# megvii-research/basedet

Measured on AMD Instinct MI355X. Metric: images/sec training RetinaNet-R50-FPN 1333x800, higher is better.
Workload: dtype bf16; 1 GPU; retinanet_r50_800x1344 train step (fwd+bwd+allreduce+SGD), DummyLoader boxes, random-init weights, inputs resident in HBM; per_gpu_batch=16, global_batch=16, parallelism=dp1

## Files before the change

basedet_amd/csrc/conv_wgrad.hip:

```cpp
#include <vector>
#include "common.h"

namespace {

constexpr int TILE = 128;
constexpr int ROW_PITCH = 288;
constexpr int MAX_SEG = BD_MAX_SEGS;

struct WSeg {
    int m_start;
    int Ho, Wo, per_img;
    float inv_per_img, inv_wo;
    int Hi, Wi, in_off, out_off;
};

struct WgradParams {
    const bf16_raw* x;
    const bf16_raw* g;
    float* slab;
    int Cin, Cout, R, S, stride, pad;
    int M, nseg;
    int in_pix_per_img, out_pix_per_img;
    int ci_tiles, co_tiles, splits, steps_per_split, total_steps;
    WSeg seg[MAX_SEG];
};

__device__ __forceinline__ void fast_divmod(int n, int d, float inv, int& q, int& r) {
    q = (int)((float)n * inv);
    r = n - q * d;
    if (r < 0) { --q; r += d; }
    else if (r >= d) { ++q; r -= d; }
}

template <int BKP, bool USE_TR>
__global__ __launch_bounds__(256) void conv_wgrad_kernel(const WgradParams p) {
    constexpr int PASSES = BKP / 16;
    constexpr int TILE_BYTES = BKP * ROW_PITCH;
    extern __shared__ __attribute__((aligned(16))) unsigned char smem[];

    const int tid = threadIdx.x;
    const int lane = tid & 63;
    const int wave = tid >> 6;
    const int wci = wave >> 1;
    const int wco = wave & 1;

    const int nwg = gridDim.x;
    int bid = blockIdx.x;
    {
        const int q = nwg >> 3, r = nwg & 7, xcd = bid & 7;
        bid = (xcd < r ? xcd * (q + 1) : r * (q + 1) + (xcd - r) * q) + (bid >> 3);
    }
    const int RS = p.R * p.S;
    const int tiles_per_split = RS * p.ci_tiles * p.co_tiles;
    const int split = bid / tiles_per_split;
    int t = bid - split * tiles_per_split;
    const int tap = t / (p.ci_tiles * p.co_tiles);
    t -= tap * (p.ci_tiles * p.co_tiles);
    const int ci_tile = t / p.co_tiles;
    const int co_tile = t - ci_tile * p.co_tiles;
    const int ci0 = ci_tile * TILE, co0 = co_tile * TILE;
    const int tap_r = tap / p.S, tap_s = tap - tap_r * p.S;

    const int step_begin = split * p.steps_per_split;
    int step_end = step_begin + p.steps_per_split;
    if (step_end > p.total_steps) step_end = p.total_steps;

    const int chunk = tid & 15;
    const int row0 = tid >> 4;
    const bool ci_ok = ci0 + chunk * 8 < p.Cin;
    const bool co_ok = co0 + chunk * 8 < p.Cout;

    u32x4_t rx[PASSES], rg[PASSES];

    auto stage_load = [&](int step) {
#pragma unroll
        for (int i = 0; i < PASSES; ++i) {
            const int m = step * BKP + row0 + i * 16;
            u32x4_t vx = {0u, 0u, 0u, 0u}, vg = {0u, 0u, 0u, 0u};
            if (m < p.M) {
                int s = 0;
#pragma unroll
                for (int k = 1; k < MAX_SEG; ++k)
                    if (k < p.nseg && m >= p.seg[k].m_start) s = k;
                const WSeg sg = p.seg[s];
                int n, rem, oy, ox;
                fast_divmod(m - sg.m_start, sg.per_img, sg.inv_per_img, n, rem);
                fast_divmod(rem, sg.Wo, sg.inv_wo, oy, ox);
                if (co_ok) {
                    const long long gp = (long long)n * p.out_pix_per_img + sg.out_off + oy * sg.Wo + ox;
                    vg = *reinterpret_cast<const u32x4_t*>(p.g + gp * p.Cout + co0 + chunk * 8);
                }
                const int sy = oy * p.stride - p.pad + tap_r, sx = ox * p.stride - p.pad + tap_s;
                if (ci_ok && sy >= 0 && sx >= 0 && sy < sg.Hi && sx < sg.Wi) {
                    const long long xp = (long long)n * p.in_pix_per_img + sg.in_off + sy * sg.Wi + sx;
                    vx = *reinterpret_cast<const u32x4_t*>(p.x + xp * p.Cin + ci0 + chunk * 8);
                }
            }
            rx[i] = vx; rg[i] = vg;
        }
    };
    auto stage_write = [&](int buf) {
        unsigned char* Xt = smem + buf * 2 * TILE_BYTES;
        unsigned char* Gt = Xt + TILE_BYTES;
#pragma unroll
        for (int i = 0; i < PASSES; ++i) {
            const int row = row0 + i * 16;
            *reinterpret_cast<u32x4_t*>(Xt + row * ROW_PITCH + chunk * 16) = rx[i];
            *reinterpret_cast<u32x4_t*>(Gt + row * ROW_PITCH + chunk * 16) = rg[i];
        }
    };

    f32x4_t acc[4][4];
#pragma unroll
    for (int i = 0; i < 4; ++i)
#pragma unroll
        for (int j = 0; j < 4; ++j) acc[i][j] = (f32x4_t){0.f, 0.f, 0.f, 0.f};

    const int g4 = lane >> 4, idx = lane & 15;
    const int prow_base = 16 * (g4 >> 1) + 4 * (g4 & 1);
    const int tr_q = idx >> 2, tr_p = idx & 3;

    auto load_frag = [&](const unsigned char* tile, int kk, int cbase) -> bf16x8_t {
        bf16x8_t f;
        if constexpr (USE_TR) {
            const unsigned char* a0 = tile + (kk * 32 + prow_base + tr_q) * ROW_PITCH + (cbase + 4 * tr_p) * 2;
            s16x4_t lo = __builtin_amdgcn_ds_read_tr16_b64_v4i16((__attribute__((address_space(3))) s16x4_t*)(a0));
            s16x4_t hi = __builtin_amdgcn_ds_read_tr16_b64_v4i16((__attribute__((address_space(3))) s16x4_t*)(a0 + 8 * ROW_PITCH));
            typedef __attribute__((ext_vector_type(8))) short s16x8_t;
            s16x8_t v = {lo[0], lo[1], lo[2], lo[3], hi[0], hi[1], hi[2], hi[3]};
            f = __builtin_bit_cast(bf16x8_t, v);
        } else {
            typedef __attribute__((ext_vector_type(8))) short s16x8_t;
            s16x8_t v;
#pragma unroll
            for (int j = 0; j < 8; ++j) {
                const int prow = kk * 32 + prow_base + (j & 3) + 8 * (j >> 2);
                v[j] = *reinterpret_cast<const short*>(tile + prow * ROW_PITCH + (cbase + idx) * 2);
            }
            f = __builtin_bit_cast(bf16x8_t, v);
        }
        return f;
    };

    auto compute = [&](int buf) {
        const unsigned char* Xt = smem + buf * 2 * TILE_BYTES;
        const unsigned char* Gt = Xt + TILE_BYTES;
#pragma unroll
        for (int kk = 0; kk < BKP / 32; ++kk) {
            bf16x8_t a[4], b[4];
#pragma unroll
            for (int i = 0; i < 4; ++i) a[i] = load_frag(Xt, kk, wci * 64 + i * 16);
#pragma unroll
            for (int j = 0; j < 4; ++j) b[j] = load_frag(Gt, kk, wco * 64 + j * 16);
#pragma unroll
            for (int i = 0; i < 4; ++i)
#pragma unroll
                for (int j = 0; j < 4; ++j)
                    acc[i][j] = __builtin_amdgcn_mfma_f32_16x16x32_bf16(a[i], b[j], acc[i][j], 0, 0, 0);
        }
    };

    if (step_begin < step_end) {
        stage_load(step_begin);
        stage_write(0);
    }
    __syncthreads();
    int cur = 0;
    for (int st = step_begin; st < step_end; ++st) {
        const bool more = st + 1 < step_end;
        if (more) stage_load(st + 1);
        compute(cur);
        if (more) stage_write(cur ^ 1);
        __syncthreads();
        cur ^= 1;
    }

    float* slab = p.slab + (long long)split * p.Cout * RS * p.Cin;
#pragma unroll
    for (int j = 0; j < 4; ++j) {
        const int co = co0 + wco * 64 + j * 16 + idx;
        if (co >= p.Cout) continue;
#pragma unroll
        for (int i = 0; i < 4; ++i) {
            const int ci = ci0 + wci * 64 + i * 16 + g4 * 4;
            if (ci >= p.Cin) continue;
            *reinterpret_cast<f32x4_t*>(slab + ((long long)co * RS + tap) * p.Cin + ci) = acc[i][j];
        }
    }
}

}
#include "wgrad_reduce.h"
namespace {

__global__ __launch_bounds__(256) void wgrad_batch_reduce_kernel(const BdRedBatch b) {
    __shared__ f32x4_t red[4][64];
    int ei = 0;
#pragma unroll 1
    for (int k = 1; k < b.count; ++k)
        if ((int)blockIdx.x >= b.e[k].block_begin) ei = k;
    const BdRedEntry& en = b.e[ei];
    const int tx = threadIdx.x & 63, ty = threadIdx.x >> 6;
    const long long e = (long long)((int)blockIdx.x - en.block_begin) * 64 + tx;
    const long long n4 = en.n4;
    f32x4_t s = {0.f, 0.f, 0.f, 0.f};
    if (e < n4) {
        const long long stride = n4 * 4;
        const float* src = en.slab + e * 4;
        const int splits = en.splits;
        int k = ty;
        for (; k + 12 < splits; k += 16) {
            const f32x4_t v0 = *reinterpret_cast<const f32x4_t*>(src + (long long)k * stride);
            const f32x4_t v1 = *reinterpret_cast<const f32x4_t*>(src + (long long)(k + 4) * stride);
            const f32x4_t v2 = *reinterpret_cast<const f32x4_t*>(src + (long long)(k + 8) * stride);
            const f32x4_t v3 = *reinterpret_cast<const f32x4_t*>(src + (long long)(k + 12) * stride);
            s += v0; s += v1; s += v2; s += v3;
        }
        for (; k < splits; k += 4) s += *reinterpret_cast<const f32x4_t*>(src + (long long)k * stride);
    }
    red[ty][tx] = s;
    __syncthreads();
    if (ty != 0 || e >= n4) return;
    f32x4_t t = red[0][tx];
    t += red[1][tx]; t += red[2][tx]; t += red[3][tx];
    long long idx;
    int row;
    if (en.kind == 0) {
        idx = e * 4;
        row = (int)(idx / en.row_len);
    } else {
        const int regs = en.regs;
        const long long per_tile = 8ll * regs * 64;
        const int tile = (int)(e / per_tile);
        int r = (int)(e - tile * per_tile);
        const int wave = r / (regs * 64);
        r -= wave * (regs * 64);
        const int reg = r >> 6, lane = r & 63;
        const int ci_tile = tile / en.co_tiles, co_tile = tile - ci_tile * en.co_tiles;
        int co, ci, tap = 0, taps = 1;
        if (en.kind == 1) {
            tap = reg >> 2; taps = 9;
            co = co_tile * en.tco + (wave >> 2) * 64 + (reg & 3) * 16 + (lane & 15);
            ci = ci_tile * en.tci + (wave & 3) * 16 + (lane >> 4) * 4;
        } else {
            const int i = reg / en.fj, j = reg - i * en.fj;
            const int wco_n = en.tco / (16 * en.fj);
            const int wci = wave / wco_n, wco = wave - wci * wco_n;
            co = co_tile * en.tco + (wco * en.fj + j) * 16 + (lane & 15);
            ci = ci_tile * en.tci + (wci * en.fi + i) * 16 + (lane >> 4) * 4;
        }
        if (co >= en.Cout || ci >= en.Cin) return;
        idx = ((long long)co * taps + tap) * en.Cin + ci;
        row = co;
    }
    float* d = en.dw + idx;
    if (en.row_scale) t *= en.row_scale[row];
    if (en.accumulate) t += *reinterpret_cast<const f32x4_t*>(d);
    *reinterpret_cast<f32x4_t*>(d) = t;
}

int launch_batch(const BdRedEntry* entries, int count, hipStream_t stream) {
    for (int base = 0; base < count; base += BD_RED_MAX) {
        BdRedBatch b{};
        b.count = count - base < BD_RED_MAX ? count - base : BD_RED_MAX;
        int blocks = 0;
        for (int k = 0; k < b.count; ++k) {
            b.e[k] = entries[base + k];
            b.e[k].block_begin = blocks;
            blocks += (int)cdiv64(b.e[k].n4, 64);
        }
        if (blocks > 0) hipLaunchKernelGGL(wgrad_batch_reduce_kernel, dim3(blocks), dim3(256), 0, stream, b);
    }
    return 0;
}

BdRedEntry plain_entry(const float* slab, int splits, long long n, int row_len, const float* row_scale, float* dw, int accumulate) {
    BdRedEntry e{};
    e.slab = slab; e.dw = dw; e.row_scale = row_scale; e.kind = 0; e.splits = splits; e.accumulate = accumulate;
    e.n4 = (int)(n / 4); e.row_len = row_len;
    return e;
}

struct Plan { int ci_tiles, co_tiles, splits, steps_per_split, total_steps; long long M; };

constexpr int BKP_DEFAULT = 64;
BD_KNOB int g_wgrad_use_tr = 1;
BD_KNOB int g_wgrad_use_3x3 = 1;
BD_KNOB int g_wgrad_use_ring = 1;

bool is_3x3s1(const bd_conv_desc* d) {
    if (!(d->R == 3 && d->S == 3 && (d->stride == 1 || d->stride == 2) && d->pad == 1)) return false;
    if ((long long)d->N * d->in_pix_per_img * d->Cin * 2 >= 0x7fffffffll || (long long)d->N * d->out_pix_per_img * d->Cout * 2 >= 0x7fffffffll)
        return false;
    for (int s = 0; s < d->nseg; ++s)
        if ((d->Hi[s] - 1) / d->stride + 1 != d->Ho[s] || (d->Wi[s] - 1) / d->stride + 1 != d->Wo[s]) return false;
    return true;
}

Plan make_plan(const bd_conv_desc* d) {
    Plan pl;
    long long M = 0;
    for (int s = 0; s < d->nseg; ++s) M += (long long)d->N * d->Ho[s] * d->Wo[s];
    pl.M = M;
    pl.ci_tiles = cdiv(d->Cin, TILE);
    pl.co_tiles = cdiv(d->Cout, TILE);
    pl.total_steps = (int)cdiv64(M, BKP_DEFAULT);
    const int tiles = d->R * d->S * pl.ci_tiles * pl.co_tiles;
    int splits = 1024 / tiles;
    if (splits < 1) splits = 1;
    const int max_splits = pl.total_steps / 4 > 0 ? pl.total_steps / 4 : 1;
    if (splits > max_splits) splits = max_splits;
    pl.steps_per_split = cdiv(pl.total_steps, splits);
    pl.splits = cdiv(pl.total_steps, pl.steps_per_split);
    return pl;
}

}

int bd_wgrad1x1_splits(const bd_conv_desc* d);
int bd_wgrad1x1_launch(const bd_conv_desc* d, const void* x, const void* g, float* slab, int* splits_out, hipStream_t stream);
int bd_wgrad3x3_splits(const bd_conv_desc* d, int* total_patches_out, int* patches_per_img_out);
int bd_wgrad3x3_launch(const bd_conv_desc* d, const void* x, const void* g, float* slab, float* csum, int* splits_out, hipStream_t stream);
bool bd_wgrad3x3r_eligible(const bd_conv_desc* d);
size_t bd_wgrad3x3r_slab_bytes(const bd_conv_desc* d, int* splits_out);
int bd_wgrad3x3r_launch(const bd_conv_desc* d, const void* x, const void* g, float* slab, float* csum, const int* gflags, int* splits_out,
                        hipStream_t stream);
int bd_wgrad3x3r_gskip_patches(const bd_conv_desc* d);
void bd_gskip_scan(const bd_conv_desc* d, const void* g, int ph, int pw, int* mask, hipStream_t stream);
void bd_wgrad3x3r_entry(const bd_conv_desc* d, BdRedEntry* e);
bool bd_wgrad1x1r_eligible(const bd_conv_desc* d);
size_t bd_wgrad1x1r_slab_bytes(const bd_conv_desc* d, int* splits_out);
int bd_wgrad1x1r_launch(const bd_conv_desc* d, const void* x, const void* g, float* slab, int* splits_out, hipStream_t stream);
void bd_wgrad1x1r_entry(const bd_conv_desc* d, BdRedEntry* e);

int bd_route_wgrad(int use_tr) {
    g_wgrad_use_tr = use_tr & 1;
    g_wgrad_use_3x3 = (use_tr & 2) ? 0 : 1;
    g_wgrad_use_ring = (use_tr & 4) ? 0 : 1;
    if (!(use_tr & 1)) g_wgrad_use_3x3 = 0;
    return BD_OK;
}

void bd_wgrad_reduce_launch(const float* slab, int splits, long long n, int row_len, const float* row_scale, float* dw, int accumulate,
                            hipStream_t stream) {
    const BdRedEntry e = plain_entry(slab, splits, n, row_len, row_scale, dw, accumulate);
    launch_batch(&e, 1, stream);
}

namespace {
size_t align256(size_t v) { return (v + 255) & ~size_t(255); }
int gskip_patches(const bd_conv_desc* d) {
    return d->gskip && bd_wgrad3x3r_eligible(d) ? bd_wgrad3x3r_gskip_patches(d) : 0;
}
size_t wgrad_ws_base(const bd_conv_desc* d);
}

extern "C" size_t bd_conv2d_wgrad_workspace_bytes(const bd_conv_desc* d) {
    BdRouteScope rs__(d);
    if (rs__.rc != BD_OK) return 0;
    if (!d || d->nseg < 1 || d->nseg > BD_MAX_SEGS) return 0;
    const size_t base = wgrad_ws_base(d);
    const int gp = gskip_patches(d);
    return gp > 0 ? align256(base) + (size_t)gp * sizeof(int) : base;
}

namespace {
size_t wgrad_ws_base(const bd_conv_desc* d) {
    const Plan pl = make_plan(d);
    size_t splits = (size_t)pl.splits;
    if (is_3x3s1(d)) {
        const size_t s3 = (size_t)bd_wgrad3x3_splits(d, nullptr, nullptr);
        if (s3 > splits) splits = s3;
    }
    if (d->R == 1 && d->S == 1 && d->pad == 0) {
        const size_t s1 = (size_t)bd_wgrad1x1_splits(d);
        if (s1 > splits) splits = s1;
    }
    size_t bytes = splits * d->Cout * d->R * d->S * d->Cin * sizeof(float);
    if (bd_wgrad3x3r_eligible(d)) {
        const size_t r = bd_wgrad3x3r_slab_bytes(d, nullptr);
        if (r > bytes) bytes = r;
    }
    if (bd_wgrad1x1r_eligible(d)) {
        const size_t r = bd_wgrad1x1r_slab_bytes(d, nullptr);
        if (r > bytes) bytes = r;
    }
    return bytes;
}
}

extern "C" size_t bd_colsum_workspace_bytes(int C);
extern "C" int bd_colsum_bf16(const void* g, int N, int64_t pix_per_img, int64_t off, int64_t cnt, int C, float* out, int accumulate,
                              void* ws, size_t ws_bytes, bd_stream_t stream);
struct bd_wgrad_queue { std::vector<BdRedEntry> entries; };
static int wgrad_impl(const bd_conv_desc* d, const void* x, const void* g, const float* row_scale, float* dw, float* dbias,
                      int accumulate, void* ws, size_t ws_bytes, bd_stream_t stream, bd_wgrad_queue* q);

extern "C" size_t bd_conv2d_wgrad_bias_workspace_bytes(const bd_conv_desc* d) {
    BdRouteScope rs__(d);
    if (rs__.rc != BD_OK) return 0;
    const size_t w = bd_conv2d_wgrad_workspace_bytes(d);
    if (!w) return 0;
    size_t extra = bd_colsum_workspace_bytes(d->Cout);
    if (is_3x3s1(d)) {
        const size_t s3 = (size_t)bd_wgrad3x3_splits(d, nullptr, nullptr) * d->Cout * sizeof(float);
        if (s3 > extra) extra = s3;
    }
    if (bd_wgrad3x3r_eligible(d)) {
        int sr = 1;
        (void)bd_wgrad3x3r_slab_bytes(d, &sr);
        const size_t s3 = (size_t)sr * d->Cout * sizeof(float);
        if (s3 > extra) extra = s3;
    }
    return align256(w) + extra;
}

extern "C" int bd_conv2d_wgrad_bias(const bd_conv_desc* d, const void* x, const void* g, const float* row_scale, float* dw,
                                    float* dbias, int accumulate, void* ws, size_t ws_bytes, bd_stream_t stream) {
    BD_ROUTE(d);
    BD_REQUIRE(dbias, "conv2d_wgrad_bias: null bias gradient");
    BD_REQUIRE(d != nullptr, "conv2d_wgrad_bias: null descriptor");
    const size_t need = bd_conv2d_wgrad_bias_workspace_bytes(d);
    if (ws_bytes < need) {
        bd_set_error("conv2d_wgrad_bias: workspace %zu < required %zu bytes", ws_bytes, need);
        return BD_EWORKSPACE;
    }
    return wgrad_impl(d, x, g, row_scale, dw, dbias, accumulate, ws, ws_bytes, stream, nullptr);
}

extern "C" int bd_conv2d_wgrad(const bd_conv_desc* d, const void* x, const void* g, const float* row_scale,
                               float* dw, int accumulate, void* ws, size_t ws_bytes, bd_stream_t stream) {
    BD_ROUTE(d);
    return wgrad_impl(d, x, g, row_scale, dw, nullptr, accumulate, ws, ws_bytes, stream, nullptr);
}

extern "C" int bd_wgrad_queue_create(bd_wgrad_queue_t* out) {
    BD_REQUIRE(out != nullptr, "bd_wgrad_queue_create: null argument");
    *out = new bd_wgrad_queue();
    return BD_OK;
}
extern "C" int bd_wgrad_queue_destroy(bd_wgrad_queue_t q) {
    delete q;
    return BD_OK;
}
extern "C" int bd_wgrad_queue_pending(bd_wgrad_queue_t q) { return q ? (int)q->entries.size() : 0; }
extern "C" int bd_conv2d_wgrad_queued(bd_wgrad_queue_t q, const bd_conv_desc* d, const void* x, const void* g, const float* row_scale, float* dw,
                                      float* dbias, int accumulate, void* ws, size_t ws_bytes, bd_stream_t stream) {
    BD_ROUTE(d);
    BD_REQUIRE(q != nullptr, "bd_conv2d_wgrad_queued: null queue");
    if (dbias) {
        BD_REQUIRE(d != nullptr, "conv2d_wgrad_queued: null descriptor");
        const size_t need = bd_conv2d_wgrad_bias_workspace_bytes(d);
        if (ws_bytes < need) {
            bd_set_error("conv2d_wgrad_queued: workspace %zu < required %zu bytes", ws_bytes, need);
            return BD_EWORKSPACE;
        }
    }
    return wgrad_impl(d, x, g, row_scale, dw, dbias, accumulate, ws, ws_bytes, stream, q);
}
extern "C" int bd_wgrad_queue_flush(bd_wgrad_queue_t q, bd_stream_t stream) {
    BD_REQUIRE(q != nullptr, "bd_wgrad_queue_flush: null queue");
    if (q->entries.empty()) return BD_OK;
    launch_batch(q->entries.data(), (int)q->entries.size(), (hipStream_t)stream);
    q->entries.clear();
    BD_CHECK_LAUNCH("bd_wgrad_queue_flush");
    return BD_OK;
}

static int wgrad_impl(const bd_conv_desc* d, const void* x, const void* g, const float* row_scale, float* dw, float* dbias,
                      int accumulate, void* ws, size_t ws_bytes, bd_stream_t stream, bd_wgrad_queue* q) {
    BD_REQUIRE(d && x && g && dw && ws, "conv2d_wgrad: null pointer");
    BD_REQUIRE(d->nseg >= 1 && d->nseg <= BD_MAX_SEGS, "conv2d_wgrad: nseg out of range");
    BD_REQUIRE(d->Cin % 8 == 0 && d->Cout % 8 == 0, "conv2d_wgrad: Cin=%d / Cout=%d must be multiples of 8", d->Cin, d->Cout);
    const Plan pl = make_plan(d);
    BD_REQUIRE(pl.M < (1ll << 24), "conv2d_wgrad: %lld pixels exceed the 2^24 fast-division range", pl.M);
    const size_t need = bd_conv2d_wgrad_workspace_bytes(d);
    if (ws_bytes < need) {
        bd_set_error("conv2d_wgrad: workspace %zu < required %zu bytes", ws_bytes, need);
        return BD_EWORKSPACE;
    }
    unsigned char* extra = (unsigned char*)ws + align256(need);
    auto bias_fallback = [&]() -> int {
        long long dense = 0;
        bool packed = true;
        for (int s = 0; s < d->nseg; ++s) { packed = packed && d->out_off[s] == dense; dense += (long long)d->Ho[s] * d->Wo[s]; }
        if (packed && dense == d->out_pix_per_img)
            return bd_colsum_bf16(g, 1, 0, 0, (int64_t)d->N * dense, d->Cout, dbias, accumulate, extra, bd_colsum_workspace_bytes(d->Cout), stream);
        for (int s = 0; s < d->nseg; ++s) {
            const int e = bd_colsum_bf16(g, d->N, d->out_pix_per_img, d->out_off[s], (int64_t)d->Ho[s] * d->Wo[s], d->Cout, dbias,
                                         (s > 0 || accumulate) ? 1 : 0, extra, bd_colsum_workspace_bytes(d->Cout), stream);
            if (e != BD_OK) return e;
        }
        return BD_OK;
    };
    auto finish = [&](const BdRedEntry& we, int splits, bool fused_csum) -> int {
        BdRedEntry es[2] = {we, {}};
        int n = 1;
        if (dbias && fused_csum) es[n++] = plain_entry((const float*)extra, splits, d->Cout, 1, nullptr, dbias, accumulate);
        if (q) {
            for (int k = 0; k < n; ++k) q->entries.push_back(es[k]);
        } else {
            launch_batch(es, n, (hipStream_t)stream);
            BD_CHECK_LAUNCH("bd_conv2d_wgrad(reduce)");
        }
        return (dbias && !fused_csum) ? bias_fallback() : BD_OK;
    };
    if (g_wgrad_use_3x3 && g_wgrad_use_ring && bd_wgrad3x3r_eligible(d)) {
        int splitsr = 1;
        bd_note_kernel("conv_wgrad3x3_ring_kernel");
        int* gflags = nullptr;
        if (gskip_patches(d) > 0) {
            if (d->gskip_gmap) {
                BdGskipMap gm;
                bd_gskip_map_layout(d, 0, &gm);
                BD_REQUIRE(d->gskip_gmap_bytes >= gm.ints * sizeof(int) && gm.p8 == gskip_patches(d),
                           "conv2d_wgrad: gskip_gmap %zu < required %zu bytes", (size_t)d->gskip_gmap_bytes, gm.ints * sizeof(int));
                gflags = (int*)d->gskip_gmap + gm.m8;
            } else {
                gflags = (int*)((unsigned char*)ws + align256(wgrad_ws_base(d)));
                bd_gskip_scan(d, g, 8, 8, gflags, (hipStream_t)stream);
            }
        }
        bd_wgrad3x3r_launch(d, x, g, (float*)ws, dbias ? (float*)extra : nullptr, gflags, &splitsr, (hipStream_t)stream);
        BD_CHECK_LAUNCH("bd_conv2d_wgrad(3x3 ring)");
        BdRedEntry e{};
        bd_wgrad3x3r_entry(d, &e);
        e.slab = (const float*)ws; e.splits = splitsr; e.row_scale = row_scale; e.dw = dw; e.accumulate = accumulate;
        return finish(e, splitsr, true);
    }
    if (g_wgrad_use_3x3 && is_3x3s1(d)) {
        int splits3 = 1;
        bd_note_kernel("conv_wgrad3x3_kernel");
        bd_wgrad3x3_launch(d, x, g, (float*)ws, dbias ? (float*)extra : nullptr, &splits3, (hipStream_t)stream);
        BD_CHECK_LAUNCH("bd_conv2d_wgrad(3x3)");
        return finish(plain_entry((const float*)ws, splits3, (long long)d->Cout * 9 * d->Cin, 9 * d->Cin, row_scale, dw, accumulate), splits3, true);
    }
    if (g_wgrad_use_3x3 && g_wgrad_use_ring && bd_wgrad1x1r_eligible(d)) {
        int splitsr = 1;
        bd_note_kernel("conv_wgrad1x1_ring_kernel");
        bd_wgrad1x1r_launch(d, x, g, (float*)ws, &splitsr, (hipStream_t)stream);
        BD_CHECK_LAUNCH("bd_conv2d_wgrad(1x1 ring)");
        BdRedEntry e{};
        bd_wgrad1x1r_entry(d, &e);
        e.slab = (const float*)ws; e.splits = splitsr; e.row_scale = row_scale; e.dw = dw; e.accumulate = accumulate;
        return finish(e, splitsr, false);
    }
    if (g_wgrad_use_3x3 && d->R == 1 && d->S == 1 && d->pad == 0) {
        int splits1 = 1;
        bd_note_kernel("conv_wgrad1x1_kernel");
        bd_wgrad1x1_launch(d, x, g, (float*)ws, &splits1, (hipStream_t)stream);
        BD_CHECK_LAUNCH("bd_conv2d_wgrad(1x1)");
        return finish(plain_entry((const float*)ws, splits1, (long long)d->Cout * d->Cin, d->Cin, row_scale, dw, accumulate), splits1, false);
    }
    WgradParams p{};
    p.x = (const bf16_raw*)x; p.g = (const bf16_raw*)g; p.slab = (float*)ws;
    p.Cin = d->Cin; p.Cout = d->Cout; p.R = d->R; p.S = d->S; p.stride = d->stride; p.pad = d->pad;
    p.M = (int)pl.M; p.nseg = d->nseg;
    p.in_pix_per_img = d->in_pix_per_img; p.out_pix_per_img = d->out_pix_per_img;
    p.ci_tiles = pl.ci_tiles; p.co_tiles = pl.co_tiles; p.splits = pl.splits;
    p.steps_per_split = pl.steps_per_split; p.total_steps = pl.total_steps;
    long long m = 0;
    for (int s = 0; s < d->nseg; ++s) {
        WSeg& sg = p.seg[s];
        sg.m_start = (int)m;
        sg.Ho = d->Ho[s]; sg.Wo = d->Wo[s]; sg.per_img = d->Ho[s] * d->Wo[s];
        sg.inv_per_img = 1.0f / (float)sg.per_img; sg.inv_wo = 1.0f / (float)sg.Wo;
        sg.Hi = d->Hi[s]; sg.Wi = d->Wi[s]; sg.in_off = d->in_off[s]; sg.out_off = d->out_off[s];
        m += (long long)d->N * sg.per_img;
    }
    const int grid = pl.splits * d->R * d->S * pl.ci_tiles * pl.co_tiles;
    const size_t lds = 4 * BKP_DEFAULT * ROW_PITCH;
    BD_ONCE_PER_DEVICE(
        (void)hipFuncSetAttribute(reinterpret_cast<const void*>(&conv_wgrad_kernel<BKP_DEFAULT, true>),
                            hipFuncAttributeMaxDynamicSharedMemorySize, (int)lds);
        (void)hipFuncSetAttribute(reinterpret_cast<const void*>(&conv_wgrad_kernel<BKP_DEFAULT, false>),
                            hipFuncAttributeMaxDynamicSharedMemorySize, (int)lds));
    bd_note_kernel("conv_wgrad_kernel");
    if (g_wgrad_use_tr)
        hipLaunchKernelGGL((conv_wgrad_kernel<BKP_DEFAULT, true>), dim3(grid), dim3(256), lds, (hipStream_t)stream, p);
    else
        hipLaunchKernelGGL((conv_wgrad_kernel<BKP_DEFAULT, false>), dim3(grid), dim3(256), lds, (hipStream_t)stream, p);
    BD_CHECK_LAUNCH("bd_conv2d_wgrad");
    const long long n = (long long)d->Cout * d->R * d->S * d->Cin;
    return finish(plain_entry((const float*)ws, pl.splits, n, d->R * d->S * d->Cin, row_scale, dw, accumulate), pl.splits, false);
}
```

basedet_amd/csrc/conv_wgrad3x3.hip:

```cpp
#include <stdlib.h>
#include "common.h"

namespace {

constexpr int PATCH = 8;
constexpr int TILE_CI = 64, TILE_CO = 64;
constexpr int X_PITCH = 160;
constexpr int G_PITCH = 160;

template <int STRIDE> struct XImg {
    static constexpr int PH = STRIDE == 1 ? PATCH : PATCH / 2, PW = PATCH;
    static constexpr int KSUB = PH / 4;
    static constexpr int XW = STRIDE == 1 ? PW + 2 : PW + 1;
    static constexpr int XH = STRIDE == 1 ? PH + 2 : PH + 1;
    static constexpr int IMG = XW * XH;
    static constexpr int ROWS = STRIDE == 1 ? IMG : 4 * IMG;
    static constexpr int X_BYTES = ROWS * X_PITCH;
    static constexpr int G_BYTES = PH * PW * G_PITCH;
    static constexpr int G_PASSES = PH * PW * 8 / 256;
    static constexpr int BUF_BYTES = X_BYTES + G_BYTES;
    static constexpr int X_CHUNKS = ROWS * 8;
    static constexpr int X_PASSES = (X_CHUNKS + 255) / 256;
    static constexpr int EXT_H = STRIDE == 1 ? PH + 2 : 2 * PH + 1;
    static constexpr int EXT_W = STRIDE == 1 ? PW + 2 : 2 * PW + 1;
    __host__ __device__ static constexpr int tap_row(int r, int s) {
        return STRIDE == 1 ? r * XW + s : ((r & 1) * 2 + (s & 1)) * IMG + (r >> 1) * XW + (s >> 1);
    }
};

struct PSeg { int patch_start, H, W, pw, in_off, out_off, Hi, Wi; };

#ifdef BD_W3_STAMP
__device__ unsigned long long g_w3_stamp[4][8];
#endif

struct W3Params {
    const bf16_raw* x;
    const bf16_raw* g;
    float* slab;
    float* csum;
    int Cin, Cout, N, nseg;
    int in_ppi, out_ppi;
    unsigned x_bytes, g_bytes;
    int patches_per_img, total_patches, patches_per_split;
    int ci_tiles, co_tiles;
    PSeg seg[BD_MAX_SEGS];
};

template <int STRIDE>
__global__ __launch_bounds__(256, 2) void conv_wgrad3x3_kernel(const W3Params p) {
    using XI = XImg<STRIDE>;
    constexpr int X_PASSES = XI::X_PASSES, X_CHUNKS = XI::X_CHUNKS, X_BYTES = XI::X_BYTES, BUF_BYTES = XI::BUF_BYTES, XW = XI::XW;
    constexpr int G_PASSES = XI::G_PASSES, PH = XI::PH, PW = XI::PW;
    extern __shared__ __attribute__((aligned(16))) unsigned char smem[];
    const int tid = threadIdx.x, lane = tid & 63, wave = tid >> 6;
    int bid = blockIdx.x;
    {
        const int nwg = gridDim.x;
        const int q = nwg >> 3, r = nwg & 7, xcd = bid & 7;
        bid = (xcd < r ? xcd * (q + 1) : r * (q + 1) + (xcd - r) * q) + (bid >> 3);
    }
    const int tiles = p.ci_tiles * p.co_tiles;
    const int split = bid / tiles;
    bid -= split * tiles;
    const int ci_tile = bid / p.co_tiles, co_tile = bid - ci_tile * p.co_tiles;
    const int ci0 = ci_tile * TILE_CI, co0 = co_tile * TILE_CO;
    const int pbeg = split * p.patches_per_split;
    int pend = pbeg + p.patches_per_split;
    if (pend > p.total_patches) pend = p.total_patches;

    int x_iy[X_PASSES], x_ix[X_PASSES];
    const int x_chunk = tid & 7;
    const bool x_cok = ci0 + x_chunk * 8 < p.Cin;
#pragma unroll
    for (int k = 0; k < X_PASSES; ++k) {
        const int c = tid + 256 * k;
        const int row = c >> 3;
        if (STRIDE == 1) {
            x_iy[k] = row < XI::ROWS ? row / XW : -1;
            x_ix[k] = row - (row / XW) * XW;
        } else {
            const int ph = row / XI::IMG, rr = row - ph * XI::IMG;
            const int a = rr / XW, b = rr - a * XW;
            const int u = 2 * a + (ph >> 1), v = 2 * b + (ph & 1);
            x_iy[k] = (row < XI::ROWS && u < XI::EXT_H && v < XI::EXT_W) ? u : -1;
            x_ix[k] = v;
        }
    }
    const int g_chunk = tid & 7;
    const bool g_cok = co0 + g_chunk * 8 < p.Cout;

    u32x4_t rx[X_PASSES], rg[G_PASSES];
    const bool do_cs = p.csum != nullptr && ci_tile == 0;
    float cs[8] = {0.f, 0.f, 0.f, 0.f, 0.f, 0.f, 0.f, 0.f};

    constexpr unsigned X_NONE = 0x80000000u;
    const __amdgpu_buffer_rsrc_t x_rsrc = __builtin_amdgcn_make_buffer_rsrc(const_cast<bf16_raw*>(p.x), 0, p.x_bytes, 0x00020000);
    const __amdgpu_buffer_rsrc_t g_rsrc = __builtin_amdgcn_make_buffer_rsrc(const_cast<bf16_raw*>(p.g), 0, p.g_bytes, 0x00020000);
    int x_vec[X_PASSES], g_vec[G_PASSES];

    int c_n = 0, c_s = 0, c_by = 0, c_bx = 0, c_rows = 1;
    PSeg sg = p.seg[0];
    auto level_vectors = [&]() {
#pragma unroll
        for (int k = 0; k < X_PASSES; ++k)
            x_vec[k] = (x_iy[k] >= 0 && x_cok) ? ((x_iy[k] * sg.Wi + x_ix[k]) * p.Cin + x_chunk * 8) * 2 : (int)X_NONE;
#pragma unroll
        for (int k = 0; k < G_PASSES; ++k) {
            const int row = (tid >> 3) + 32 * k;
            g_vec[k] = g_cok ? (((row >> 3) * sg.W + (row & 7)) * p.Cout + g_chunk * 8) * 2 : (int)X_NONE;
        }
    };
    auto seek = [&](int pid) {
        c_n = pid / p.patches_per_img;
        const int rem = pid - c_n * p.patches_per_img;
        c_s = 0;
#pragma unroll
        for (int k = 1; k < BD_MAX_SEGS; ++k)
            if (k < p.nseg && rem >= p.seg[k].patch_start) c_s = k;
        sg = p.seg[c_s];
        const int local = rem - sg.patch_start;
        c_by = local / sg.pw; c_bx = local - c_by * sg.pw;
        c_rows = (sg.H + PH - 1) / PH;
        level_vectors();
    };
    auto advance = [&]() {
        if (++c_bx < sg.pw) return;
        c_bx = 0;
        if (++c_by < c_rows) return;
        c_by = 0;
        if (p.nseg == 1) { ++c_n; return; }
        if (++c_s == p.nseg) { c_s = 0; ++c_n; }
        sg = p.seg[c_s];
        c_rows = (sg.H + PH - 1) / PH;
        level_vectors();
    };

    auto stage_load = [&]() {
        const int n = c_n, by = c_by, bx = c_bx;
        const int y0 = by * PH, x0 = bx * PW;
        const int ys = STRIDE * y0 - 1, xs = STRIDE * x0 - 1;
        const int xorg = (n * p.in_ppi + sg.in_off + ys * sg.Wi + xs) * p.Cin + ci0;
        const int gorg = (n * p.out_ppi + sg.out_off + y0 * sg.W + x0) * p.Cout + co0;
        if (ys >= 0 && xs >= 0 && ys + XI::EXT_H <= sg.Hi && xs + XI::EXT_W <= sg.Wi && y0 + PH <= sg.H && x0 + PW <= sg.W) {
#pragma unroll
            for (int k = 0; k < X_PASSES; ++k)
                rx[k] = __builtin_amdgcn_raw_buffer_load_b128(x_rsrc, (unsigned)x_vec[k], xorg * 2, 0);
#pragma unroll
            for (int k = 0; k < G_PASSES; ++k) rg[k] = __builtin_amdgcn_raw_buffer_load_b128(g_rsrc, (unsigned)g_vec[k], gorg * 2, 0);
            return;
        }
#pragma unroll
        for (int k = 0; k < X_PASSES; ++k) {
            const int y = ys + x_iy[k], x = xs + x_ix[k];
            const bool ok = x_iy[k] >= 0 && x_cok && y >= 0 && x >= 0 && y < sg.Hi && x < sg.Wi;
            rx[k] = __builtin_amdgcn_raw_buffer_load_b128(x_rsrc, ok ? (unsigned)xorg * 2u + (unsigned)x_vec[k] : X_NONE, 0, 0);
        }
#pragma unroll
        for (int k = 0; k < G_PASSES; ++k) {
            const int row = (tid >> 3) + 32 * k;
            const bool ok = g_cok && y0 + (row >> 3) < sg.H && x0 + (row & 7) < sg.W;
            rg[k] = __builtin_amdgcn_raw_buffer_load_b128(g_rsrc, ok ? (unsigned)gorg * 2u + (unsigned)g_vec[k] : X_NONE, 0, 0);
        }
    };
    auto stage_write = [&](int buf) {
        unsigned char* Xt = smem + buf * BUF_BYTES;
        unsigned char* Gt = Xt + X_BYTES;
#pragma unroll
        for (int k = 0; k < X_PASSES; ++k) {
            const int c = tid + 256 * k;
            if (256 * (k + 1) <= X_CHUNKS || c < X_CHUNKS) *reinterpret_cast<u32x4_t*>(Xt + (c >> 3) * X_PITCH + x_chunk * 16) = rx[k];
        }
#pragma unroll
        for (int k = 0; k < G_PASSES; ++k) {
            const int row = (tid >> 3) + 32 * k;
            *reinterpret_cast<u32x4_t*>(Gt + row * G_PITCH + g_chunk * 16) = rg[k];
        }
        if (do_cs) {
#pragma unroll
            for (int k = 0; k < G_PASSES; ++k)
#pragma unroll
                for (int j = 0; j < 4; ++j) { cs[2 * j] += bf_lo(rg[k][j]); cs[2 * j + 1] += bf_hi(rg[k][j]); }
        }
    };

    f32x4_t acc[9][4];
#pragma unroll
    for (int t = 0; t < 9; ++t)
#pragma unroll
        for (int j = 0; j < 4; ++j) acc[t][j] = (f32x4_t){0.f, 0.f, 0.f, 0.f};

    const int g4 = lane >> 4, idx = lane & 15;
    const int tr_q = idx >> 2, tr_p = idx & 3;
    const int prow_hi = 2 * (g4 >> 1);
    const int pcol = 4 * (g4 & 1) + tr_q;
    const int x_lane_off = (prow_hi * XW + pcol) * X_PITCH + (wave * 16 + 4 * tr_p) * 2;
    const int g_lane_off = (prow_hi * PW + pcol) * G_PITCH + (4 * tr_p) * 2;

    typedef __attribute__((ext_vector_type(8))) short s16x8_t;
    auto tr_frag = [&](const unsigned char* a0, int row_pitch_bytes) -> bf16x8_t {
        const s16x4_t lo = __builtin_amdgcn_ds_read_tr16_b64_v4i16((__attribute__((address_space(3))) s16x4_t*)(a0));
        const s16x4_t hi = __builtin_amdgcn_ds_read_tr16_b64_v4i16((__attribute__((address_space(3))) s16x4_t*)(a0 + row_pitch_bytes));
        const s16x8_t v = {lo[0], lo[1], lo[2], lo[3], hi[0], hi[1], hi[2], hi[3]};
        return __builtin_bit_cast(bf16x8_t, v);
    };

    auto compute = [&](int buf) {
        const unsigned char* Xt = smem + buf * BUF_BYTES + x_lane_off;
        const unsigned char* Gt = smem + buf * BUF_BYTES + X_BYTES + g_lane_off;
        constexpr int NT = 9 * XI::KSUB;
        bf16x8_t a[2], b[2][4];
#pragma unroll
        for (int j = 0; j < 4; ++j) b[0][j] = tr_frag(Gt + j * 32, PW * G_PITCH);
        a[0] = tr_frag(Xt + XI::tap_row(0, 0) * X_PITCH, XW * X_PITCH);
        __builtin_amdgcn_sched_barrier(0);
        __builtin_amdgcn_s_setprio(1);
#pragma unroll
        for (int i = 0; i < NT; ++i) {
            const int kk = i / 9, t = i % 9;
            if (i + 1 < NT) {
                const int k2 = (i + 1) / 9, t2 = (i + 1) % 9;
                a[(i + 1) & 1] = tr_frag(Xt + (4 * k2 * XW + XI::tap_row(t2 / 3, t2 % 3)) * X_PITCH, XW * X_PITCH);
            }
            if (kk + 1 < XI::KSUB && t >= 1 && t <= 4)
                b[(kk + 1) & 1][t - 1] = tr_frag(Gt + (4 * (kk + 1) * PW) * G_PITCH + (t - 1) * 32, PW * G_PITCH);
            __builtin_amdgcn_sched_barrier(0);
#pragma unroll
            for (int j = 0; j < 4; ++j)
                acc[t][j] = __builtin_amdgcn_mfma_f32_16x16x32_bf16(a[i & 1], b[kk & 1][j], acc[t][j], 0, 0, 0);
            __builtin_amdgcn_sched_barrier(0);
        }
        __builtin_amdgcn_s_setprio(0);
    };

    if (pbeg < pend) {
        seek(pbeg);
        stage_load();
        advance();
        stage_write(0);
    }
    __syncthreads();
    int cur = 0;
#ifdef BD_W3_STAMP
    unsigned long long st[5] = {0, 0, 0, 0, 0};
    const unsigned long long st_begin = __builtin_amdgcn_s_memtime();
    const unsigned long long st_rbegin = __builtin_amdgcn_s_memrealtime();
#define W3_T() __builtin_amdgcn_s_memtime()
    for (int pid = pbeg; pid < pend; ++pid) {
        const bool more = pid + 1 < pend;
        const unsigned long long a0 = W3_T();
        if (more) { stage_load(); advance(); }
        __builtin_amdgcn_sched_barrier(0);
        const unsigned long long a1 = W3_T();
        compute(cur);
        __builtin_amdgcn_sched_barrier(0);
        const unsigned long long a2 = W3_T();
        if (more) stage_write(cur ^ 1);
        asm volatile("s_waitcnt lgkmcnt(0)" ::: "memory");
        const unsigned long long a3 = W3_T();
        __syncthreads();
        const unsigned long long a4 = W3_T();
        st[0] += a1 - a0; st[1] += a2 - a1; st[2] += a3 - a2; st[3] += a4 - a3; st[4] += 1;
        cur ^= 1;
    }
    if (blockIdx.x == 300 % gridDim.x && lane == 0) {
        for (int k = 0; k < 5; ++k) g_w3_stamp[wave][k] = st[k];
        g_w3_stamp[wave][5] = __builtin_amdgcn_s_memtime() - st_begin;
        g_w3_stamp[wave][6] = __builtin_amdgcn_s_memrealtime() - st_rbegin;
    }
#else
    for (int pid = pbeg; pid < pend; ++pid) {
        const bool more = pid + 1 < pend;
        if (more) { stage_load(); advance(); }
        compute(cur);
        if (more) stage_write(cur ^ 1);
        __syncthreads();
        cur ^= 1;
    }
#endif

    if (do_cs) {
        float* red = reinterpret_cast<float*>(smem);
#pragma unroll
        for (int j = 0; j < 8; ++j) red[tid * 8 + j] = cs[j];
        __syncthreads();
        if (tid < TILE_CO && co0 + tid < p.Cout) {
            float s = 0.f;
            for (int r = 0; r < 32; ++r) s += red[(r * 8 + (tid >> 3)) * 8 + (tid & 7)];
            p.csum[(long long)split * p.Cout + co0 + tid] = s;
        }
    }
    float* slab = p.slab + (long long)split * p.Cout * 9 * p.Cin;
#pragma unroll
    for (int j = 0; j < 4; ++j) {
        const int co = co0 + j * 16 + idx;
        if (co >= p.Cout) continue;
        const int ci = ci0 + wave * 16 + g4 * 4;
        if (ci >= p.Cin) continue;
#pragma unroll
        for (int t = 0; t < 9; ++t)
            *reinterpret_cast<f32x4_t*>(slab + ((long long)co * 9 + t) * p.Cin + ci) = acc[t][j];
    }
}

}

int bd_wgrad3x3_splits(const bd_conv_desc* d, int* total_patches_out, int* patches_per_img_out) {
    int ppi = 0;
    const int ph = d->stride == 1 ? XImg<1>::PH : XImg<2>::PH;
    for (int s = 0; s < d->nseg; ++s) ppi += cdiv(d->Ho[s], ph) * cdiv(d->Wo[s], PATCH);
    const int total = ppi * d->N;
    const int tiles = cdiv(d->Cin, TILE_CI) * cdiv(d->Cout, TILE_CO);
    static const int target = bd_tune_env("BD_WGRAD3_TARGET", 512);
    int splits = target / tiles;
    if (splits < 1) splits = 1;
    if (splits > total) splits = total;
    const int per = cdiv(total, splits);
    splits = cdiv(total, per);
    if (total_patches_out) *total_patches_out = total;
    if (patches_per_img_out) *patches_per_img_out = ppi;
    return splits;
}

#ifdef BD_W3_STAMP
extern "C" int bd_debug_w3_stamp(unsigned long long* out32) {
    return hipMemcpyFromSymbol(out32, HIP_SYMBOL(g_w3_stamp), sizeof(g_w3_stamp)) == hipSuccess ? 0 : 1;
}
#endif

int bd_wgrad3x3_launch(const bd_conv_desc* d, const void* x, const void* g, float* slab, float* csum, int* splits_out, hipStream_t stream) {
    W3Params p{};
    p.x = (const bf16_raw*)x; p.g = (const bf16_raw*)g; p.slab = slab; p.csum = csum;
    p.Cin = d->Cin; p.Cout = d->Cout; p.N = d->N; p.nseg = d->nseg;
    p.in_ppi = d->in_pix_per_img; p.out_ppi = d->out_pix_per_img;
    p.x_bytes = (unsigned)((long long)d->N * d->in_pix_per_img * d->Cin * 2);
    p.g_bytes = (unsigned)((long long)d->N * d->out_pix_per_img * d->Cout * 2);
    int total, ppi;
    const int splits = bd_wgrad3x3_splits(d, &total, &ppi);
    p.total_patches = total; p.patches_per_img = ppi; p.patches_per_split = cdiv(total, splits);
    p.ci_tiles = cdiv(d->Cin, TILE_CI); p.co_tiles = cdiv(d->Cout, TILE_CO);
    int ps = 0;
    const int ph = d->stride == 1 ? XImg<1>::PH : XImg<2>::PH;
    for (int s = 0; s < d->nseg; ++s) {
        PSeg& sg = p.seg[s];
        sg.patch_start = ps; sg.H = d->Ho[s]; sg.W = d->Wo[s]; sg.pw = cdiv(d->Wo[s], PATCH);
        sg.in_off = d->in_off[s]; sg.out_off = d->out_off[s]; sg.Hi = d->Hi[s]; sg.Wi = d->Wi[s];
        ps += cdiv(d->Ho[s], ph) * sg.pw;
    }
    BD_ONCE_PER_DEVICE(
        (void)hipFuncSetAttribute(reinterpret_cast<const void*>(&conv_wgrad3x3_kernel<1>), hipFuncAttributeMaxDynamicSharedMemorySize,
                                  2 * XImg<1>::BUF_BYTES);
        (void)hipFuncSetAttribute(reinterpret_cast<const void*>(&conv_wgrad3x3_kernel<2>), hipFuncAttributeMaxDynamicSharedMemorySize,
                                  2 * XImg<2>::BUF_BYTES));
    const int grid = splits * p.ci_tiles * p.co_tiles;
    if (d->stride == 1) hipLaunchKernelGGL(conv_wgrad3x3_kernel<1>, dim3(grid), dim3(256), 2 * XImg<1>::BUF_BYTES, stream, p);
    else hipLaunchKernelGGL(conv_wgrad3x3_kernel<2>, dim3(grid), dim3(256), 2 * XImg<2>::BUF_BYTES, stream, p);
    *splits_out = splits;
    return 0;
}
```

Measured before the change: 721.6 images/sec.

## Add LDS-DMA triple-buffered pipeline to stride-2 3x3 weight-gradient kernel

Adds a variant of the stride-2 3x3 wgrad kernel that loads input and gradient patches straight into LDS with buffer_load ... lds, skipping the register staging. It uses a 3-stage ring with prefetch depth 2, counted vmcnt waits and an XOR-swizzled 128-byte row layout that replaces the padded pitch. This is meant to cut VGPR pressure and register-to-LDS copy instructions and to overlap global loads with MFMA compute. The risks are more LDS per workgroup, fragile counted waits that depend on how many pieces each wave issues, and inline asm. The new path is on by default and can be turned off with a routing bit.

```diff
diff --git a/basedet_amd/csrc/conv_wgrad.hip b/basedet_amd/csrc/conv_wgrad.hip
--- a/basedet_amd/csrc/conv_wgrad.hip
+++ b/basedet_amd/csrc/conv_wgrad.hip
@@ -333,7 +333,9 @@
 int bd_wgrad1x1r_launch(const bd_conv_desc* d, const void* x, const void* g, float* slab, int* splits_out, hipStream_t stream);
 void bd_wgrad1x1r_entry(const bd_conv_desc* d, BdRedEntry* e);
 
+BD_KNOB int g_wgrad_s2_dma = 1;
 int bd_route_wgrad(int use_tr) {
+    g_wgrad_s2_dma = (use_tr & 8) ? 0 : 1;
     g_wgrad_use_tr = use_tr & 1;
     g_wgrad_use_3x3 = (use_tr & 2) ? 0 : 1;
     g_wgrad_use_ring = (use_tr & 4) ? 0 : 1;
diff --git a/basedet_amd/csrc/conv_wgrad3x3.hip b/basedet_amd/csrc/conv_wgrad3x3.hip
--- a/basedet_amd/csrc/conv_wgrad3x3.hip
+++ b/basedet_amd/csrc/conv_wgrad3x3.hip
@@ -28,6 +28,30 @@
     }
 };
 
+struct DmaS2 {
+    static constexpr int ROW = 128;
+    static constexpr int X_ROWS = XImg<2>::ROWS;
+    static constexpr int X_PIECES = (X_ROWS + 7) / 8;
+    static constexpr int X_BYTES = X_ROWS * ROW;
+    static constexpr int G_BYTES = XImg<2>::PH * XImg<2>::PW * ROW;
+    static constexpr int STAGE = X_BYTES + G_BYTES;
+    static constexpr int NSTAGE = 3, DEPTH = 2;
+    static constexpr int LDS_BYTES = NSTAGE * STAGE;
+    static constexpr int NXP = (X_PIECES + 3) / 4;
+    __host__ __device__ static constexpr int piece_row(int pc) { return pc == X_PIECES - 1 ? X_ROWS - 8 : 8 * pc; }
+};
+static_assert(2 * DmaS2::LDS_BYTES <= 160 * 1024, "two workgroups per CU");
+static_assert(DmaS2::X_PIECES % 4 == 3, "waves 0 .. 2 issue NXP X pieces, wave 3 one fewer (the counted waits below)");
+
+typedef __attribute__((address_space(3))) void lds_void_w3_t;
+
+__device__ __forceinline__ void w3_dma16(__amdgpu_buffer_rsrc_t rsrc, unsigned lds_addr, unsigned voff, int soff) {
+    asm volatile("s_mov_b32 m0, %1\n\ts_nop 0\n\tbuffer_load_dwordx4 %0, %2, %3 offen lds" : : "v"(voff), "s"(lds_addr), "s"(rsrc), "s"(soff) : "memory");
+}
+__device__ __forceinline__ void w3_dma16(__amdgpu_buffer_rsrc_t rsrc, unsigned lds_addr, unsigned voff) {
+    asm volatile("s_mov_b32 m0, %1\n\ts_nop 0\n\tbuffer_load_dwordx4 %0, %2, 0 offen lds" : : "v"(voff), "s"(lds_addr), "s"(rsrc) : "memory");
+}
+
 struct PSeg { int patch_start, H, W, pw, in_off, out_off, Hi, Wi; };
 
 #ifdef BD_W3_STAMP
@@ -47,13 +71,14 @@
     PSeg seg[BD_MAX_SEGS];
 };
 
-template <int STRIDE>
+template <int STRIDE, bool DMA>
 __global__ __launch_bounds__(256, 2) void conv_wgrad3x3_kernel(const W3Params p) {
+    static_assert(!DMA || STRIDE == 2, "the LDS-DMA ring serves the stride-2 instance");
     using XI = XImg<STRIDE>;
     constexpr int X_PASSES = XI::X_PASSES, X_CHUNKS = XI::X_CHUNKS, X_BYTES = XI::X_BYTES, BUF_BYTES = XI::BUF_BYTES, XW = XI::XW;
     constexpr int G_PASSES = XI::G_PASSES, PH = XI::PH, PW = XI::PW;
     extern __shared__ __attribute__((aligned(16))) unsigned char smem[];
-    const int tid = threadIdx.x, lane = tid & 63, wave = tid >> 6;
+    const int tid = threadIdx.x, lane = tid & 63, wave = DMA ? __builtin_amdgcn_readfirstlane(tid >> 6) : tid >> 6;
     int bid = blockIdx.x;
     {
         const int nwg = gridDim.x;
@@ -99,9 +124,39 @@
     const __amdgpu_buffer_rsrc_t g_rsrc = __builtin_amdgcn_make_buffer_rsrc(const_cast<bf16_raw*>(p.g), 0, p.g_bytes, 0x00020000);
     int x_vec[X_PASSES], g_vec[G_PASSES];
 
+    using DS = DmaS2;
+    int d_iy[DS::NXP], d_ix[DS::NXP];
+    unsigned d_xin[DS::NXP], d_gin = X_NONE;
+    const int d_gx = lane >> 3;
+    const int d_gcb = ((lane & 7) ^ (2 * ((d_gx >> 1) & 3))) * 16;
+    const bool d_gok = co0 + (d_gcb >> 1) < p.Cout;
+    if constexpr (DMA) {
+#pragma unroll
+        for (int k = 0; k < DS::NXP; ++k) {
+            const int pc = wave + 4 * k;
+            const int row = DS::piece_row(pc) + (lane >> 3);
+            const int ph = row / XI::IMG, rr = row - ph * XI::IMG;
+            const int a = rr / XW, b = rr - a * XW;
+            const int u = 2 * a + (ph >> 1), v = 2 * b + (ph & 1);
+            const int c = (lane & 7) ^ (2 * ((b >> 1) & 3));
+            d_iy[k] = (pc < DS::X_PIECES && u < XI::EXT_H && v < XI::EXT_W && ci0 + c * 8 < p.Cin) ? u : -1;
+            d_ix[k] = v;
+        }
+    }
+    const unsigned lds0 = __builtin_amdgcn_readfirstlane((unsigned)reinterpret_cast<uintptr_t>((lds_void_w3_t*)smem));
+
     int c_n = 0, c_s = 0, c_by = 0, c_bx = 0, c_rows = 1;
     PSeg sg = p.seg[0];
     auto level_vectors = [&]() {
+        if constexpr (DMA) {
+#pragma unroll
+            for (int k = 0; k < DS::NXP; ++k) {
+                const int cb = ((lane & 7) ^ (2 * ((d_ix[k] >> 2) & 3))) * 16;
+                d_xin[k] = d_iy[k] >= 0 ? (unsigned)(((d_iy[k] * sg.Wi + d_ix[k]) * p.Cin) * 2 + cb) : X_NONE;
+            }
+            d_gin = d_gok ? (unsigned)(((wave * sg.W + d_gx) * p.Cout) * 2 + d_gcb) : X_NONE;
+            return;
+        }
 #pragma unroll
         for (int k = 0; k < X_PASSES; ++k)
             x_vec[k] = (x_iy[k] >= 0 && x_cok) ? ((x_iy[k] * sg.Wi + x_ix[k]) * p.Cin + x_chunk * 8) * 2 : (int)X_NONE;
@@ -121,6 +176,11 @@
         sg = p.seg[c_s];
         const int local = rem - sg.patch_start;
         c_by = local / sg.pw; c_bx = local - c_by * sg.pw;
+        if constexpr (DMA) {
+            c_n = __builtin_amdgcn_readfirstlane(c_n);
+            c_by = __builtin_amdgcn_readfirstlane(c_by);
+            c_bx = __builtin_amdgcn_readfirstlane(c_bx);
+        }
         c_rows = (sg.H + PH - 1) / PH;
         level_vectors();
     };
@@ -184,6 +244,35 @@
         }
     };
 
+    auto dma_issue = [&](int stage, bool dead) {
+        const unsigned Xs = __builtin_amdgcn_readfirstlane(lds0 + stage * DS::STAGE);
+        const int y0 = c_by * PH, x0 = c_bx * PW;
+        const int ys = STRIDE * y0 - 1, xs = STRIDE * x0 - 1;
+        const int xorg = __builtin_amdgcn_readfirstlane(((c_n * p.in_ppi + sg.in_off + ys * sg.Wi + xs) * p.Cin + ci0) * 2);
+        const int gorg = __builtin_amdgcn_readfirstlane(((c_n * p.out_ppi + sg.out_off + y0 * sg.W + x0) * p.Cout + co0) * 2);
+        if (!dead && ys >= 0 && xs >= 0 && ys + XI::EXT_H <= sg.Hi && xs + XI::EXT_W <= sg.Wi) {
+#pragma unroll
+            for (int k = 0; k < DS::NXP; ++k) {
+                if (k == DS::NXP - 1 && wave == 3) break;
+                w3_dma16(x_rsrc, Xs + DS::piece_row(wave + 4 * k) * DS::ROW, d_xin[k], xorg);
+            }
+        } else {
+#pragma unroll
+            for (int k = 0; k < DS::NXP; ++k) {
+                if (k == DS::NXP - 1 && wave == 3) break;
+                const bool ok = !dead & (d_iy[k] >= 0) & ((unsigned)(ys + d_iy[k]) < (unsigned)sg.Hi) & ((unsigned)(xs + d_ix[k]) < (unsigned)sg.Wi);
+                w3_dma16(x_rsrc, Xs + DS::piece_row(wave + 4 * k) * DS::ROW, ok ? (unsigned)xorg + d_xin[k] : X_NONE);
+            }
+        }
+        const unsigned Gs = Xs + DS::X_BYTES + wave * 1024;
+        if (!dead && y0 + PH <= sg.H && x0 + PW <= sg.W) {
+            w3_dma16(g_rsrc, Gs, d_gin, gorg);
+        } else {
+            const bool ok = !dead & d_gok & (y0 + wave < sg.H) & (x0 + d_gx < sg.W);
+            w3_dma16(g_rsrc, Gs, ok ? (unsigned)gorg + d_gin : X_NONE);
+        }
+    };
+
     f32x4_t acc[9][4];
 #pragma unroll
     for (int t = 0; t < 9; ++t)
@@ -196,6 +285,13 @@
     const int pcol = 4 * (g4 & 1) + tr_q;
     const int x_lane_off = (prow_hi * XW + pcol) * X_PITCH + (wave * 16 + 4 * tr_p) * 2;
     const int g_lane_off = (prow_hi * PW + pcol) * G_PITCH + (4 * tr_p) * 2;
+    int xa[2], ga[4];
+#pragma unroll
+    for (int sc = 0; sc < 2; ++sc)
+        xa[sc] = (prow_hi * XW + pcol + sc) * DS::ROW + ((wave ^ (((pcol + sc) >> 1) & 3)) * 32) + tr_p * 8;
+#pragma unroll
+    for (int j = 0; j < 4; ++j)
+        ga[j] = DS::X_BYTES + (prow_hi * PW + pcol) * DS::ROW + ((j ^ ((pcol >> 1) & 3)) * 32) + tr_p * 8;
 
     typedef __attribute__((ext_vector_type(8))) short s16x8_t;
     auto tr_frag = [&](const unsigned char* a0, int row_pitch_bytes) -> bf16x8_t {
@@ -208,11 +304,20 @@
     auto compute = [&](int buf) {
         const unsigned char* Xt = smem + buf * BUF_BYTES + x_lane_off;
         const unsigned char* Gt = smem + buf * BUF_BYTES + X_BYTES + g_lane_off;
+        const unsigned char* St = smem + buf * DS::STAGE;
         constexpr int NT = 9 * XI::KSUB;
+        auto x_frag = [&](int kk, int r, int s) -> bf16x8_t {
+            if constexpr (DMA) return tr_frag(St + xa[s >> 1] + (XI::tap_row(r, s) - (s >> 1)) * DS::ROW, XW * DS::ROW);
+            else return tr_frag(Xt + (4 * kk * XW + XI::tap_row(r, s)) * X_PITCH, XW * X_PITCH);
+        };
+        auto g_frag = [&](int kk, int j) -> bf16x8_t {
+            if constexpr (DMA) return tr_frag(St + ga[j], PW * DS::ROW);
+            else return tr_frag(Gt + (4 * kk * PW) * G_PITCH + j * 32, PW * G_PITCH);
+        };
         bf16x8_t a[2], b[2][4];
 #pragma unroll
-        for (int j = 0; j < 4; ++j) b[0][j] = tr_frag(Gt + j * 32, PW * G_PITCH);
-        a[0] = tr_frag(Xt + XI::tap_row(0, 0) * X_PITCH, XW * X_PITCH);
+        for (int j = 0; j < 4; ++j) b[0][j] = g_frag(0, j);
+        a[0] = x_frag(0, 0, 0);
         __builtin_amdgcn_sched_barrier(0);
         __builtin_amdgcn_s_setprio(1);
 #pragma unroll
@@ -220,10 +325,10 @@
             const int kk = i / 9, t = i % 9;
             if (i + 1 < NT) {
                 const int k2 = (i + 1) / 9, t2 = (i + 1) % 9;
-                a[(i + 1) & 1] = tr_frag(Xt + (4 * k2 * XW + XI::tap_row(t2 / 3, t2 % 3)) * X_PITCH, XW * X_PITCH);
+                a[(i + 1) & 1] = x_frag(k2, t2 / 3, t2 % 3);
             }
             if (kk + 1 < XI::KSUB && t >= 1 && t <= 4)
-                b[(kk + 1) & 1][t - 1] = tr_frag(Gt + (4 * (kk + 1) * PW) * G_PITCH + (t - 1) * 32, PW * G_PITCH);
+                b[(kk + 1) & 1][t - 1] = g_frag(kk + 1, t - 1);
             __builtin_amdgcn_sched_barrier(0);
 #pragma unroll
             for (int j = 0; j < 4; ++j)
@@ -233,6 +338,46 @@
         __builtin_amdgcn_s_setprio(0);
     };
 
+    if constexpr (DMA) {
+#define W3_WAIT_NEXT() do { if (wave == 3) asm volatile("s_waitcnt vmcnt(%0)" :: "n"(DS::NXP) : "memory"); \
+                            else asm volatile("s_waitcnt vmcnt(%0)" :: "n"(DS::NXP + 1) : "memory"); } while (0)
+#define W3_BARRIER() do { asm volatile("s_waitcnt lgkmcnt(0)" ::: "memory"); __builtin_amdgcn_s_barrier(); asm volatile("" ::: "memory"); } while (0)
+        const int nsteps = __builtin_amdgcn_readfirstlane(pend > pbeg ? pend - pbeg : 0);
+        if (nsteps > 0) {
+            seek(pbeg);
+#pragma unroll 1
+            for (int d = 0; d < DS::DEPTH; ++d) {
+                dma_issue(d, d >= nsteps);
+                advance();
+            }
+            W3_WAIT_NEXT();
+            W3_BARRIER();
+            int stage = 0, fill = DS::DEPTH;
+#pragma unroll 1
+            for (int t = 0; t < nsteps; ++t) {
+                dma_issue(fill, t + DS::DEPTH >= nsteps);
+                advance();
+                __builtin_amdgcn_sched_barrier(0);
+                compute(stage);
+                if (do_cs) {
+                    const int row = tid >> 3;
+                    const u32x4_t v = *reinterpret_cast<const u32x4_t*>(smem + stage * DS::STAGE + DS::X_BYTES + row * DS::ROW +
+                                                                        (((tid & 7) ^ (2 * (((row & 7) >> 1) & 3))) * 16));
+#pragma unroll
+                    for (int j = 0; j < 4; ++j) { cs[2 * j] += bf_lo(v[j]); cs[2 * j + 1] += bf_hi(v[j]); }
+                }
+                __builtin_amdgcn_sched_barrier(0);
+                W3_WAIT_NEXT();
+                W3_BARRIER();
+                stage = stage + 1 == DS::NSTAGE ? 0 : stage + 1;
+                fill = fill + 1 == DS::NSTAGE ? 0 : fill + 1;
+            }
+            asm volatile("s_waitcnt vmcnt(0)" ::: "memory");
+        }
+        __syncthreads();
+#undef W3_WAIT_NEXT
+#undef W3_BARRIER
+    } else {
     if (pbeg < pend) {
         seek(pbeg);
         stage_load();
@@ -278,6 +423,7 @@
         cur ^= 1;
     }
 #endif
+    }
 
     if (do_cs) {
         float* red = reinterpret_cast<float*>(smem);
@@ -304,6 +450,8 @@
 }
 
 }
+
+extern BD_KNOB int g_wgrad_s2_dma;
 
 int bd_wgrad3x3_splits(const bd_conv_desc* d, int* total_patches_out, int* patches_per_img_out) {
     int ppi = 0;
@@ -348,13 +496,21 @@
         ps += cdiv(d->Ho[s], ph) * sg.pw;
     }
     BD_ONCE_PER_DEVICE(
-        (void)hipFuncSetAttribute(reinterpret_cast<const void*>(&conv_wgrad3x3_kernel<1>), hipFuncAttributeMaxDynamicSharedMemorySize,
+        (void)hipFuncSetAttribute(reinterpret_cast<const void*>(&conv_wgrad3x3_kernel<1, false>), hipFuncAttributeMaxDynamicSharedMemorySize,
                                   2 * XImg<1>::BUF_BYTES);
-        (void)hipFuncSetAttribute(reinterpret_cast<const void*>(&conv_wgrad3x3_kernel<2>), hipFuncAttributeMaxDynamicSharedMemorySize,
-                                  2 * XImg<2>::BUF_BYTES));
+        (void)hipFuncSetAttribute(reinterpret_cast<const void*>(&conv_wgrad3x3_kernel<2, false>), hipFuncAttributeMaxDynamicSharedMemorySize,
+                                  2 * XImg<2>::BUF_BYTES);
+        (void)hipFuncSetAttribute(reinterpret_cast<const void*>(&conv_wgrad3x3_kernel<2, true>), hipFuncAttributeMaxDynamicSharedMemorySize,
+                                  DmaS2::LDS_BYTES));
     const int grid = splits * p.ci_tiles * p.co_tiles;
-    if (d->stride == 1) hipLaunchKernelGGL(conv_wgrad3x3_kernel<1>, dim3(grid), dim3(256), 2 * XImg<1>::BUF_BYTES, stream, p);
-    else hipLaunchKernelGGL(conv_wgrad3x3_kernel<2>, dim3(grid), dim3(256), 2 * XImg<2>::BUF_BYTES, stream, p);
+#ifdef BD_W3_STAMP
+    const bool dma = false;
+#else
+    const bool dma = g_wgrad_s2_dma != 0;
+#endif
+    if (d->stride == 1) hipLaunchKernelGGL((conv_wgrad3x3_kernel<1, false>), dim3(grid), dim3(256), 2 * XImg<1>::BUF_BYTES, stream, p);
+    else if (dma) hipLaunchKernelGGL((conv_wgrad3x3_kernel<2, true>), dim3(grid), dim3(256), DmaS2::LDS_BYTES, stream, p);
+    else hipLaunchKernelGGL((conv_wgrad3x3_kernel<2, false>), dim3(grid), dim3(256), 2 * XImg<2>::BUF_BYTES, stream, p);
     *splits_out = splits;
     return 0;
 }
```

Result: no change. 725.2 images/sec (median of 6 runs) (+0.5%).
